# bdaiinstitute/vlfm

Hardware: NVIDIA H100
Metric: value-map steps/sec (ITM+cone-fuse) (higher is better)
Workload: dtype f16

## Files before the change

vlfm_b200/csrc/common.cuh:

```cuda
#pragma once
#include <cuda_fp16.h>
#include <cuda_runtime.h>
#include <stdint.h>
#include <stdio.h>

#include "../../include/vlfm_b200.h"

namespace vlfm {

void set_error(const char* fmt, ...);
void count_launch(unsigned n = 1);

inline int check_cuda(cudaError_t e, const char* what) {
  if (e != cudaSuccess) {
    set_error("%s: %s", what, cudaGetErrorString(e));
    return VLFM_E_CUDA;
  }
  return VLFM_OK;
}

#define VLFM_CHECK_LAUNCH(what)                                   \
  do {                                                            \
    int _rc = ::vlfm::check_cuda(cudaGetLastError(), what);       \
    if (_rc != VLFM_OK) return _rc;                               \
  } while (0)

__device__ __forceinline__ void pdl_trigger() { asm volatile("griddepcontrol.launch_dependents;" ::: "memory"); }
__device__ __forceinline__ void pdl_wait() { asm volatile("griddepcontrol.wait;" ::: "memory"); }

bool pdl_enabled();

template <typename... KArgs, typename... Args>
inline cudaError_t launch_pdl(void (*kernel)(KArgs...), dim3 grid, dim3 block, size_t smem, cudaStream_t st, Args&&... args) {
  cudaLaunchConfig_t cfg{};
  cfg.gridDim = grid; cfg.blockDim = block; cfg.dynamicSmemBytes = smem; cfg.stream = st;
  cudaLaunchAttribute attr[1];
  attr[0].id = cudaLaunchAttributeProgrammaticStreamSerialization;
  attr[0].val.programmaticStreamSerializationAllowed = 1;
  cfg.attrs = attr; cfg.numAttrs = pdl_enabled() ? 1 : 0;
  return cudaLaunchKernelEx(&cfg, kernel, static_cast<KArgs>(args)...);
}

constexpr float X2_SCALE = 2048.f;
__device__ __forceinline__ void split_x2(float y, __half& hi, __half& lo) {
  hi = __float2half_rn(y);
  lo = __float2half_rn((y - __half2float(hi)) * X2_SCALE);
}
constexpr int SK_TILE = 128;
constexpr int SK_SLAB_ROWS = SK_TILE + 2;
constexpr long long SK_SLAB = (long long)SK_SLAB_ROWS * SK_TILE;
struct SplitK {
  int splits;
  long long stride;
  int ctas, row_tiles, tiles, num_k;
  __host__ __device__ __forceinline__ int sk_begin(int c) const { return (int)((long long)c * tiles * num_k / ctas); }
  __host__ __device__ __forceinline__ int sk_owner(int it) const { return (int)(((long long)(it + 1) * ctas - 1) / ((long long)tiles * num_k)); }
};

constexpr int LN_DMAX = 1536;
int layernorm_check(const char* who, const float* d_x, const float* d_gamma, const float* d_beta, const void* d_out16, const void* d_out16_lo,
                    const float* d_out32, int D, int ldx, int ldo16, int ldo32);

__device__ __forceinline__ float ld_cg_f32(const float* p) { return __ldcg(p); }
__device__ __forceinline__ uint32_t ld_cg_u32(const uint32_t* p) { return __ldcg(p); }

}
```

vlfm_b200/csrc/gemm_wgmma.cu:

```cuda
#include <cuda.h>
#include <cuda_fp16.h>
#include <math.h>
#include <stdlib.h>

#include "common.cuh"

namespace vlfm {

constexpr int BM = 128;
constexpr int BK = 64;
constexpr int GEMM_THREADS = 384;
constexpr int GEMM_CONSUMERS = 256;

__device__ __forceinline__ uint32_t smem_u32(const void* p) { return (uint32_t)__cvta_generic_to_shared(p); }

__device__ __forceinline__ void mbar_init(uint32_t bar, uint32_t count) {
  asm volatile("mbarrier.init.shared::cta.b64 [%0], %1;" ::"r"(bar), "r"(count));
}
__device__ __forceinline__ void mbar_expect_tx(uint32_t bar, uint32_t bytes) {
  asm volatile("mbarrier.arrive.expect_tx.shared::cta.b64 _, [%0], %1;" ::"r"(bar), "r"(bytes) : "memory");
}
__device__ __forceinline__ void mbar_arrive(uint32_t bar) {
  asm volatile("mbarrier.arrive.shared::cta.b64 _, [%0];" ::"r"(bar) : "memory");
}
__device__ __forceinline__ void mbar_wait(uint32_t bar, uint32_t parity) {
  uint32_t done = 0;
  for (uint32_t spin = 0; !done; ++spin) {
    asm volatile(
        "{\n\t.reg .pred p;\n\t"
        "mbarrier.try_wait.parity.shared::cta.b64 p, [%1], %2;\n\t"
        "selp.u32 %0, 1, 0, p;\n\t}"
        : "=r"(done) : "r"(bar), "r"(parity) : "memory");
    if (spin > (1u << 26)) __trap();
  }
}
__device__ __forceinline__ void tma_load_2d(uint32_t dst, const CUtensorMap* map, int x, int y, uint32_t bar) {
  asm volatile(
      "cp.async.bulk.tensor.2d.shared::cluster.global.mbarrier::complete_tx::bytes [%0], [%1, {%3, %4}], [%2];"
      ::"r"(dst), "l"(map), "r"(bar), "r"(x), "r"(y) : "memory");
}
__device__ __forceinline__ uint64_t wgmma_desc_k128(uint32_t saddr) {
  return (uint64_t)((saddr & 0x3FFFF) >> 4) | ((uint64_t)1 << 16) | ((uint64_t)(1024 >> 4) << 32) | ((uint64_t)1 << 62);
}
__device__ __forceinline__ void wg_fence() { asm volatile("wgmma.fence.sync.aligned;" ::: "memory"); }
__device__ __forceinline__ void wg_commit() { asm volatile("wgmma.commit_group.sync.aligned;" ::: "memory"); }
template <int PENDING>
__device__ __forceinline__ void wg_wait() { asm volatile("wgmma.wait_group.sync.aligned %0;" ::"n"(PENDING) : "memory"); }

#define VLFM_D4(d, i) "+f"(d[i]), "+f"(d[i + 1]), "+f"(d[i + 2]), "+f"(d[i + 3])
#define VLFM_D16(d, i) VLFM_D4(d, i), VLFM_D4(d, i + 4), VLFM_D4(d, i + 8), VLFM_D4(d, i + 12)
template <int BN> struct Wgmma;
template <> struct Wgmma<32> {
  static __device__ __forceinline__ void mma(float (&d)[16], uint64_t a, uint64_t b, uint32_t acc) {
    asm volatile(
        "{\n\t.reg .pred p;\n\tsetp.ne.b32 p, %18, 0;\n\t"
        "wgmma.mma_async.sync.aligned.m64n32k16.f32.f16.f16 "
        "{%0,%1,%2,%3,%4,%5,%6,%7,%8,%9,%10,%11,%12,%13,%14,%15}, %16, %17, p, 1, 1, 0, 0;\n\t}"
        : VLFM_D16(d, 0) : "l"(a), "l"(b), "r"(acc));
  }
};
template <> struct Wgmma<64> {
  static __device__ __forceinline__ void mma(float (&d)[32], uint64_t a, uint64_t b, uint32_t acc) {
    asm volatile(
        "{\n\t.reg .pred p;\n\tsetp.ne.b32 p, %34, 0;\n\t"
        "wgmma.mma_async.sync.aligned.m64n64k16.f32.f16.f16 "
        "{%0,%1,%2,%3,%4,%5,%6,%7,%8,%9,%10,%11,%12,%13,%14,%15,"
        "%16,%17,%18,%19,%20,%21,%22,%23,%24,%25,%26,%27,%28,%29,%30,%31}, %32, %33, p, 1, 1, 0, 0;\n\t}"
        : VLFM_D16(d, 0), VLFM_D16(d, 16) : "l"(a), "l"(b), "r"(acc));
  }
};
template <> struct Wgmma<96> {
  static __device__ __forceinline__ void mma(float (&d)[48], uint64_t a, uint64_t b, uint32_t acc) {
    asm volatile(
        "{\n\t.reg .pred p;\n\tsetp.ne.b32 p, %50, 0;\n\t"
        "wgmma.mma_async.sync.aligned.m64n96k16.f32.f16.f16 "
        "{%0,%1,%2,%3,%4,%5,%6,%7,%8,%9,%10,%11,%12,%13,%14,%15,"
        "%16,%17,%18,%19,%20,%21,%22,%23,%24,%25,%26,%27,%28,%29,%30,%31,"
        "%32,%33,%34,%35,%36,%37,%38,%39,%40,%41,%42,%43,%44,%45,%46,%47}, %48, %49, p, 1, 1, 0, 0;\n\t}"
        : VLFM_D16(d, 0), VLFM_D16(d, 16), VLFM_D16(d, 32) : "l"(a), "l"(b), "r"(acc));
  }
};
template <> struct Wgmma<128> {
  static __device__ __forceinline__ void mma(float (&d)[64], uint64_t a, uint64_t b, uint32_t acc) {
    asm volatile(
        "{\n\t.reg .pred p;\n\tsetp.ne.b32 p, %66, 0;\n\t"
        "wgmma.mma_async.sync.aligned.m64n128k16.f32.f16.f16 "
        "{%0,%1,%2,%3,%4,%5,%6,%7,%8,%9,%10,%11,%12,%13,%14,%15,"
        "%16,%17,%18,%19,%20,%21,%22,%23,%24,%25,%26,%27,%28,%29,%30,%31,"
        "%32,%33,%34,%35,%36,%37,%38,%39,%40,%41,%42,%43,%44,%45,%46,%47,"
        "%48,%49,%50,%51,%52,%53,%54,%55,%56,%57,%58,%59,%60,%61,%62,%63}, %64, %65, p, 1, 1, 0, 0;\n\t}"
        : VLFM_D16(d, 0), VLFM_D16(d, 16), VLFM_D16(d, 32), VLFM_D16(d, 48) : "l"(a), "l"(b), "r"(acc));
  }
};
#undef VLFM_D16
#undef VLFM_D4

struct GemmArgs {
  const float* bias;
  void* out;
  int M, N, K, ldo, epi;
  int kb_per_split;
  long long split_stride;
  const __half* a_tail; int lda, tail_rows, tail_row0;
  void* out_lo;
  int a_box_rows;
  SplitK sk;
};
constexpr int GEMM_TAIL_MAX = 2;
static_assert(SK_SLAB_ROWS == BM + GEMM_TAIL_MAX && SK_TILE == BM, "stream-K slab = one 128 x 128 tile + its tail rows");
constexpr int GEMM_TAIL_KMAX = 6144;

__device__ __forceinline__ float gelu_erf(float x) { return 0.5f * x * (1.f + erff(x * 0.70710678118654752f)); }
__device__ __forceinline__ float silu(float x) { return x / (1.f + expf(-x)); }

__device__ __forceinline__ void epilogue_store2(const GemmArgs& g, int row, int n, float v0, float v1, bool pair, bool split) {
  const size_t idx = (size_t)row * g.ldo + n;
  if (g.epi == VLFM_EPI_BIAS_F16 || g.epi == VLFM_EPI_BIAS_GELU_F16 || g.epi == VLFM_EPI_BIAS_RELU_F16 || g.epi == VLFM_EPI_BIAS_GELU_F16X2) {
// ... 963 lines not shown
```

vlfm_b200/csrc/vit_ops.cu:

```cuda
#include <cuda_fp16.h>
#include <math.h>

#include "common.cuh"

namespace vlfm {

__device__ __forceinline__ uint8_t clip8(int v) {
  v >>= 22;
  return (uint8_t)(v < 0 ? 0 : (v > 255 ? 255 : v));
}

__global__ void resize_h_kernel(const uint8_t* __restrict__ in, uint8_t* __restrict__ mid, int H, int W, int OW,
                                const int* __restrict__ bounds, const int* __restrict__ kk, int ksize) {
  const int b = blockIdx.z, y = blockIdx.y;
  const int i = blockIdx.x * blockDim.x + threadIdx.x;
  if (i >= OW * 3) return;
  const int xo = i / 3, c = i - 3 * xo;
  const int x0 = bounds[2 * xo], n = bounds[2 * xo + 1];
  const uint8_t* row = in + ((size_t)b * H + y) * W * 3;
  int ss = 1 << 21;
  for (int t = 0; t < n; ++t) ss += (int)row[(x0 + t) * 3 + c] * kk[xo * ksize + t];
  mid[(((size_t)b * H + y) * OW + xo) * 3 + c] = clip8(ss);
}

__global__ void resize_v_norm_im2col_kernel(const uint8_t* __restrict__ mid, __half* __restrict__ out, int H, int OW,
                                            int OH, const int* __restrict__ bounds, const int* __restrict__ kk,
                                            int ksize, int patch, int ldk, float m0, float m1, float m2, float s0,
                                            float s1, float s2) {
  const int b = blockIdx.z, yo = blockIdx.y;
  const int i = blockIdx.x * blockDim.x + threadIdx.x;
  if (i >= OW * 3) return;
  const int xo = i / 3, c = i - 3 * xo;
  const int y0 = bounds[2 * yo], n = bounds[2 * yo + 1];
  int ss = 1 << 21;
  for (int t = 0; t < n; ++t) ss += (int)mid[(((size_t)b * H + y0 + t) * OW + xo) * 3 + c] * kk[yo * ksize + t];
  const float px = (float)clip8(ss);
  const float mean = c == 0 ? m0 : (c == 1 ? m1 : m2), sd = c == 0 ? s0 : (c == 1 ? s1 : s2);
  const float v = __fdiv_rn(__fsub_rn(__fdiv_rn(px, 255.f), mean), sd);
  const int gp = OW / patch;
  const int py = yo / patch, ky = yo - py * patch, pxi = xo / patch, kx = xo - pxi * patch;
  const size_t rowi = (size_t)b * (OH / patch) * gp + (size_t)py * gp + pxi;
  out[rowi * ldk + c * patch * patch + ky * patch + kx] = __float2half_rn(v);
}

__global__ void assemble_tokens_kernel(const float* __restrict__ patch, const float* __restrict__ cls,
                                       const float* __restrict__ pos, float* __restrict__ x, int B, int T, int D) {
  const size_t n = (size_t)B * T * D;
  for (size_t i = (size_t)blockIdx.x * blockDim.x + threadIdx.x; i < n; i += (size_t)gridDim.x * blockDim.x) {
    const int d = (int)(i % D);
    const size_t r = i / D;
    const int t = (int)(r % T), b = (int)(r / T);
    float v = t == 0 ? cls[d] : patch[((size_t)b * (T - 1) + (t - 1)) * D + d];
    x[i] = v + pos[(size_t)t * D + d];
  }
}

template <int MAXV4>
__global__ void __launch_bounds__(128)
layernorm_kernel(const float* __restrict__ x, const float* __restrict__ gamma, const float* __restrict__ beta,
                 __half* __restrict__ out16, float* __restrict__ out32, int rows, int D, int ldx, int ldo16, int ldo32,
                 float eps, __half* __restrict__ out16_lo) {
  pdl_trigger();
  const int row = blockIdx.x * 4 + (threadIdx.x >> 5), lane = threadIdx.x & 31;
  const int D4 = D >> 2;
  float4 g[MAXV4], bt[MAXV4], v[MAXV4];
#pragma unroll
  for (int i = 0; i < MAXV4; ++i) {
    const int j = lane + 32 * i;
    g[i] = j < D4 ? __ldg(reinterpret_cast<const float4*>(gamma) + j) : make_float4(0, 0, 0, 0);
    bt[i] = j < D4 ? __ldg(reinterpret_cast<const float4*>(beta) + j) : make_float4(0, 0, 0, 0);
  }
  pdl_wait();
  if (row >= rows) return;
  const float4* xr = reinterpret_cast<const float4*>(x + (size_t)row * ldx);
  float s = 0.f;
#pragma unroll
  for (int i = 0; i < MAXV4; ++i) {
    const int j = lane + 32 * i;
    v[i] = j < D4 ? xr[j] : make_float4(0, 0, 0, 0);
    s += (v[i].x + v[i].y) + (v[i].z + v[i].w);
  }
#pragma unroll
  for (int o = 16; o; o >>= 1) s += __shfl_xor_sync(0xffffffffu, s, o);
  const float mean = s / (float)D;
// ... 52 lines not shown
    s1 = sk.sk_owner((tile + 1) * sk.num_k - 1) + tile + 1;
    stride = SK_SLAB;
    off = (long long)(row - m * SK_TILE) * SK_TILE + (4 * t - nb * SK_TILE);
  }
  pdl_wait();
  float4* xr = reinterpret_cast<float4*>(x + (size_t)row * ldx);
  float4 v = on ? xr[t] : make_float4(0, 0, 0, 0);
  for (int sp0 = s0; sp0 < s1; sp0 += 4) {
    float4 pv[4];
#pragma unroll
    for (int u = 0; u < 4; ++u) {
      const float4* pr = reinterpret_cast<const float4*>(partials + (size_t)(sp0 + u) * (size_t)stride + (size_t)off);
      pv[u] = (sp0 + u < s1 && on) ? __ldcg(pr) : make_float4(0, 0, 0, 0);
    }
#pragma unroll
    for (int u = 0; u < 4; ++u)
      if (sp0 + u < s1) { v.x += pv[u].x; v.y += pv[u].y; v.z += pv[u].z; v.w += pv[u].w; }
  }
  float s = 0.f;
  if (on) { xr[t] = v; s = (v.x + v.y) + (v.z + v.w); }
#pragma unroll
  for (int o = 16; o; o >>= 1) s += __shfl_xor_sync(0xffffffffu, s, o);
  if (lane == 0) red[0][w] = s;
  __syncthreads();
  float tot = 0.f;
  for (int i = 0; i < nw; ++i) tot += red[0][i];
  const float mean = tot / (float)D;
  float q = 0.f;
  if (on) { const float a = v.x - mean, b = v.y - mean, c = v.z - mean, d = v.w - mean; q = (a * a + b * b) + (c * c + d * d); }
#pragma unroll
  for (int o = 16; o; o >>= 1) q += __shfl_xor_sync(0xffffffffu, q, o);
  if (lane == 0) red[1][w] = q;
  __syncthreads();
  float qt = 0.f;
  for (int i = 0; i < nw; ++i) qt += red[1][i];
  const float rstd = rsqrtf(qt / (float)D + eps);
  if (on) {
    float4 y;
    y.x = (v.x - mean) * rstd * g.x + bt.x;
    y.y = (v.y - mean) * rstd * g.y + bt.y;
    y.z = (v.z - mean) * rstd * g.z + bt.z;
    y.w = (v.w - mean) * rstd * g.w + bt.w;
    if (out16) {
      __half2 h0 = __floats2half2_rn(y.x, y.y), h1 = __floats2half2_rn(y.z, y.w);
      uint2 pk = make_uint2(*reinterpret_cast<uint32_t*>(&h0), *reinterpret_cast<uint32_t*>(&h1));
      *reinterpret_cast<uint2*>(out16 + (size_t)row * ldo16 + 4 * t) = pk;
      if (out16_lo) {
        const float2 f0 = __half22float2(h0), f1 = __half22float2(h1);
        __half2 l0 = __floats2half2_rn((y.x - f0.x) * X2_SCALE, (y.y - f0.y) * X2_SCALE), l1 = __floats2half2_rn((y.z - f1.x) * X2_SCALE, (y.w - f1.y) * X2_SCALE);
        uint2 pl = make_uint2(*reinterpret_cast<uint32_t*>(&l0), *reinterpret_cast<uint32_t*>(&l1));
        *reinterpret_cast<uint2*>(out16_lo + (size_t)row * ldo16 + 4 * t) = pl;
      }
    }
    if (out32) *reinterpret_cast<float4*>(out32 + (size_t)row * ldo32 + 4 * t) = y;
  }
}

__device__ __forceinline__ void mma_16816(float (&c)[4], const uint32_t (&a)[4], uint32_t b0, uint32_t b1) {
  asm volatile(
      "mma.sync.aligned.m16n8k16.row.col.f32.f16.f16.f32 {%0,%1,%2,%3}, {%4,%5,%6,%7}, {%8,%9}, {%0,%1,%2,%3};"
      : "+f"(c[0]), "+f"(c[1]), "+f"(c[2]), "+f"(c[3])
      : "r"(a[0]), "r"(a[1]), "r"(a[2]), "r"(a[3]), "r"(b0), "r"(b1));
}
__device__ __forceinline__ uint32_t pack_half2(float a, float b) {
  __half2 h = __floats2half2_rn(a, b);
  return *reinterpret_cast<uint32_t*>(&h);
}

struct AttnArgs {
  const __half* q; const __half* k; const __half* v; __half* o;
  int ldq, ldk, ldv, ldo;
  int Nq, Nk, hd, heads;
  float scale_log2;
};

constexpr int ATT_WARPS = 4;
constexpr int ATT_NKMAX = 272;

__device__ __forceinline__ void ldmatrix_x2_trans(uint32_t& r0, uint32_t& r1, const __half* p) {
  uint32_t addr = (uint32_t)__cvta_generic_to_shared(p);
  asm volatile("ldmatrix.sync.aligned.m8n8.x2.trans.shared.b16 {%0,%1}, [%2];" : "=r"(r0), "=r"(r1) : "r"(addr));
}

template <int HDP, int KH>
__global__ void __launch_bounds__(32 * (KH == 4 ? 8 : ATT_WARPS))
attention_kernel(AttnArgs a) {
  constexpr int NW = KH == 4 ? 8 : ATT_WARPS;
  constexpr int RG = NW / KH;
  constexpr int ATT_QBLK = 16 * RG;
  constexpr int KS = HDP + 8;
  extern __shared__ __align__(16) uint8_t att_smem[];
  __half* sK = reinterpret_cast<__half*>(att_smem);
  const int b = blockIdx.z, h = blockIdx.y, qb = blockIdx.x;
  const int tid = threadIdx.x, warp = tid >> 5, lane = tid & 31, g = lane >> 2, t = lane & 3;
  const int NKP = (a.Nk + 15) & ~15;
  __half* sV = sK + NKP * KS;
  pdl_trigger();
  pdl_wait();
  const __half* kbase = a.k + (size_t)b * a.Nk * a.ldk + (size_t)h * a.hd;
  const __half* vbase = a.v + (size_t)b * a.Nk * a.ldv + (size_t)h * a.hd;

  constexpr int CH = HDP / 8;
  for (int i = tid; i < NKP * CH; i += 32 * NW) {
    const int key = i / CH, c = (i - key * CH) * 8;
    const bool ok = key < a.Nk && c < a.hd;
    const __half* ksrc = ok ? kbase + (size_t)key * a.ldk + c : kbase;
    const __half* vsrc = ok ? vbase + (size_t)key * a.ldv + c : vbase;
    const uint32_t kd = (uint32_t)__cvta_generic_to_shared(sK + key * KS + c), vd = (uint32_t)__cvta_generic_to_shared(sV + key * KS + c);
    const int nbytes = ok ? 16 : 0;
    asm volatile("cp.async.cg.shared.global [%0], [%1], 16, %2;" ::"r"(kd), "l"(ksrc), "r"(nbytes) : "memory");
    asm volatile("cp.async.cg.shared.global [%0], [%1], 16, %2;" ::"r"(vd), "l"(vsrc), "r"(nbytes) : "memory");
  }
  asm volatile("cp.async.commit_group;" ::: "memory");

  const int row0 = qb * ATT_QBLK + (warp % RG) * 16;
  const int r_lo = row0 + g, r_hi = row0 + g + 8;
  const __half* qlo = a.q + ((size_t)b * a.Nq + r_lo) * a.ldq + (size_t)h * a.hd;
  const __half* qhi = a.q + ((size_t)b * a.Nq + r_hi) * a.ldq + (size_t)h * a.hd;
  uint32_t qf[HDP / 16][4];
#pragma unroll
  for (int kk = 0; kk < HDP / 16; ++kk) {
    const int c0 = kk * 16 + 2 * t, c1 = c0 + 8;
    qf[kk][0] = (r_lo < a.Nq && c0 < a.hd) ? *reinterpret_cast<const uint32_t*>(qlo + c0) : 0u;
    qf[kk][1] = (r_hi < a.Nq && c0 < a.hd) ? *reinterpret_cast<const uint32_t*>(qhi + c0) : 0u;
    qf[kk][2] = (r_lo < a.Nq && c1 < a.hd) ? *reinterpret_cast<const uint32_t*>(qlo + c1) : 0u;
    qf[kk][3] = (r_hi < a.Nq && c1 < a.hd) ? *reinterpret_cast<const uint32_t*>(qhi + c1) : 0u;
  }
  asm volatile("cp.async.wait_group 0;" ::: "memory");
  __syncthreads();

  float o[HDP / 8][4];
#pragma unroll
  for (int i = 0; i < HDP / 8; ++i) { o[i][0] = o[i][1] = o[i][2] = o[i][3] = 0.f; }
  float m_lo = -INFINITY, m_hi = -INFINITY, l_lo = 0.f, l_hi = 0.f;

  const int part = warp / RG, tiles = NKP >> 4, tbase = tiles / KH, trem = tiles % KH;
  const int k_begin = 16 * (part * tbase + min(part, trem)), k_end = k_begin + 16 * (tbase + (part < trem ? 1 : 0));
  for (int kb = k_begin; kb < k_end; kb += 64) {
    const int ntiles = min(8, (k_end - kb) >> 3);
    float s[8][4];
#pragma unroll
    for (int j = 0; j < 8; ++j) {
      s[j][0] = s[j][1] = s[j][2] = s[j][3] = 0.f;
      if (j < ntiles) {
        const __half* kr = sK + (kb + j * 8 + g) * KS + 2 * t;
#pragma unroll
        for (int kk = 0; kk < HDP / 16; ++kk) {
          uint32_t b0 = *reinterpret_cast<const uint32_t*>(kr + kk * 16);
          uint32_t b1 = *reinterpret_cast<const uint32_t*>(kr + kk * 16 + 8);
          mma_16816(s[j], qf[kk], b0, b1);
        }
      }
    }
    float bm_lo = -INFINITY, bm_hi = -INFINITY;
#pragma unroll
    for (int j = 0; j < 8; ++j) {
      const int key = kb + j * 8 + 2 * t;
#pragma unroll
      for (int e = 0; e < 4; ++e) {
        const bool ok = (j < ntiles) && (key + (e & 1) < a.Nk);
        s[j][e] = ok ? s[j][e] * a.scale_log2 : -INFINITY;
      }
      bm_lo = fmaxf(bm_lo, fmaxf(s[j][0], s[j][1]));
      bm_hi = fmaxf(bm_hi, fmaxf(s[j][2], s[j][3]));
    }
    bm_lo = fmaxf(bm_lo, __shfl_xor_sync(0xffffffffu, bm_lo, 1));
    bm_lo = fmaxf(bm_lo, __shfl_xor_sync(0xffffffffu, bm_lo, 2));
    bm_hi = fmaxf(bm_hi, __shfl_xor_sync(0xffffffffu, bm_hi, 1));
    bm_hi = fmaxf(bm_hi, __shfl_xor_sync(0xffffffffu, bm_hi, 2));
    const float mn_lo = fmaxf(m_lo, bm_lo), mn_hi = fmaxf(m_hi, bm_hi);
    const float ref_lo = mn_lo == -INFINITY ? 0.f : mn_lo, ref_hi = mn_hi == -INFINITY ? 0.f : mn_hi;
    const float al_lo = exp2f(m_lo - ref_lo), al_hi = exp2f(m_hi - ref_hi);
    m_lo = mn_lo; m_hi = mn_hi;
    float sum_lo = 0.f, sum_hi = 0.f;
#pragma unroll
    for (int j = 0; j < 8; ++j) {
      s[j][0] = exp2f(s[j][0] - ref_lo); s[j][1] = exp2f(s[j][1] - ref_lo);
      s[j][2] = exp2f(s[j][2] - ref_hi); s[j][3] = exp2f(s[j][3] - ref_hi);
      sum_lo += s[j][0] + s[j][1]; sum_hi += s[j][2] + s[j][3];
    }
    l_lo = l_lo * al_lo + sum_lo; l_hi = l_hi * al_hi + sum_hi;
#pragma unroll
    for (int i = 0; i < HDP / 8; ++i) { o[i][0] *= al_lo; o[i][1] *= al_lo; o[i][2] *= al_hi; o[i][3] *= al_hi; }
#pragma unroll
    for (int p = 0; p < 4; ++p) {
      if (2 * p < ntiles) {
        uint32_t pa[4];
        pa[0] = pack_half2(s[2 * p][0], s[2 * p][1]);
        pa[1] = pack_half2(s[2 * p][2], s[2 * p][3]);
        pa[2] = pack_half2(s[2 * p + 1][0], s[2 * p + 1][1]);
        pa[3] = pack_half2(s[2 * p + 1][2], s[2 * p + 1][3]);
        const __half* vr = sV + (kb + p * 16 + (lane & 15)) * KS;
#pragma unroll
        for (int i = 0; i < HDP / 8; ++i) {
          uint32_t b0, b1;
          ldmatrix_x2_trans(b0, b1, vr + i * 8);
          mma_16816(o[i], pa, b0, b1);
        }
      }
    }
  }
  l_lo += __shfl_xor_sync(0xffffffffu, l_lo, 1); l_lo += __shfl_xor_sync(0xffffffffu, l_lo, 2);
  l_hi += __shfl_xor_sync(0xffffffffu, l_hi, 1); l_hi += __shfl_xor_sync(0xffffffffu, l_hi, 2);

  if (KH == 1) {
    const float inv_lo = 1.f / l_lo, inv_hi = 1.f / l_hi;
    __half* olo = a.o + ((size_t)b * a.Nq + r_lo) * a.ldo + (size_t)h * a.hd;
    __half* ohi = a.o + ((size_t)b * a.Nq + r_hi) * a.ldo + (size_t)h * a.hd;
#pragma unroll
    for (int i = 0; i < HDP / 8; ++i) {
      const int c = i * 8 + 2 * t;
      if (c < a.hd) {
        if (r_lo < a.Nq) *reinterpret_cast<uint32_t*>(olo + c) = pack_half2(o[i][0] * inv_lo, o[i][1] * inv_lo);
        if (r_hi < a.Nq) *reinterpret_cast<uint32_t*>(ohi + c) = pack_half2(o[i][2] * inv_hi, o[i][3] * inv_hi);
      }
    }
    return;
  }
  __syncthreads();
  float* mrg = reinterpret_cast<float*>(att_smem);
  constexpr int MW = HDP / 8 * 4 + 4;
  if (warp >= RG) {
// ... 236 lines not shown

namespace vlfm {
int layernorm_check(const char* who, const float* d_x, const float* d_gamma, const float* d_beta, const void* d_out16, const void* d_out16_lo,
                    const float* d_out32, int D, int ldx, int ldo16, int ldo32) {
  if (D > LN_DMAX) { set_error("%s: D=%d too large (max %d)", who, D, LN_DMAX); return VLFM_E_UNSUPPORTED; }
  if ((D & 3) || (ldx & 3) || (ldo16 & 3) || (ldo32 & 3)) { set_error("%s: D and strides must be multiples of 4", who); return VLFM_E_UNSUPPORTED; }
  if (((uintptr_t)d_x & 15) || ((uintptr_t)d_gamma & 15) || ((uintptr_t)d_beta & 15) || ((uintptr_t)d_out32 & 15) ||
      ((uintptr_t)d_out16 & 7) || ((uintptr_t)d_out16_lo & 7)) {
    set_error("%s: x, gamma, beta, out32 must be 16-byte aligned, the fp16 outputs 8-byte aligned", who); return VLFM_E_INVALID; }
  return VLFM_OK;
}
}

static int layernorm_impl(const float* d_x, const float* d_gamma, const float* d_beta, void* d_out16, void* d_out16_lo, float* d_out32,
                          int rows, int D, int ldx, int ldo16, int ldo32, float eps, void* stream) {
  __half* lo16 = (__half*)d_out16_lo;
  if (!d_x || !d_gamma || !d_beta || (!d_out16 && !d_out32) || rows < 1 || D < 1) { set_error("vlfm_layernorm: bad argument"); return VLFM_E_INVALID; }
  if (int rc = layernorm_check("vlfm_layernorm", d_x, d_gamma, d_beta, d_out16, d_out16_lo, d_out32, D, ldx, ldo16, ldo32)) return rc;
  cudaStream_t st = (cudaStream_t)stream;
  const dim3 grid((rows + 3) / 4);
  cudaError_t e;
  __half* o16 = (__half*)d_out16;
  if (D <= 128 * 2) e = launch_pdl(layernorm_kernel<2>, grid, dim3(128), 0, st, d_x, d_gamma, d_beta, o16, d_out32, rows, D, ldx, ldo16, ldo32, eps, lo16);
  else if (D <= 128 * 6) e = launch_pdl(layernorm_kernel<6>, grid, dim3(128), 0, st, d_x, d_gamma, d_beta, o16, d_out32, rows, D, ldx, ldo16, ldo32, eps, lo16);
  else e = launch_pdl(layernorm_kernel<12>, grid, dim3(128), 0, st, d_x, d_gamma, d_beta, o16, d_out32, rows, D, ldx, ldo16, ldo32, eps, lo16);
  { int rc = check_cuda(e, "layernorm_kernel"); if (rc) return rc; }
  count_launch();
  return VLFM_OK;
}
extern "C" int vlfm_layernorm(const float* d_x, const float* d_gamma, const float* d_beta, void* d_out16, float* d_out32,
                              int rows, int D, int ldx, int ldo16, int ldo32, float eps, void* stream) {
  return layernorm_impl(d_x, d_gamma, d_beta, d_out16, nullptr, d_out32, rows, D, ldx, ldo16, ldo32, eps, stream);
}
extern "C" int vlfm_layernorm_x2(const float* d_x, const float* d_gamma, const float* d_beta, void* d_out_hi, void* d_out_lo, float* d_out32,
                                 int rows, int D, int ldx, int ldo16, int ldo32, float eps, void* stream) {
  if (!d_out_hi || !d_out_lo) { set_error("vlfm_layernorm_x2: null output"); return VLFM_E_INVALID; }
  return layernorm_impl(d_x, d_gamma, d_beta, d_out_hi, d_out_lo, d_out32, rows, D, ldx, ldo16, ldo32, eps, stream);
}

namespace vlfm {
int layernorm_reduce_impl(float* d_x, const float* d_partials, const SplitK& sk, const float* d_gamma,
                          const float* d_beta, void* d_out16, void* d_out16_lo, float* d_out32, int rows, int D, int ldx, int ldo16, int ldo32,
                          float eps, void* stream) {
  __half* lo16 = (__half*)d_out16_lo;
  if (!d_x || !d_partials || !d_gamma || !d_beta || (!d_out16 && !d_out32) || rows < 1 || D < 1 || sk.splits < 0 || sk.splits > 16 ||
      (sk.splits == 0 && (sk.ctas < 1 || sk.row_tiles < 1 || sk.tiles != sk.row_tiles * ((D + SK_TILE - 1) / SK_TILE) || sk.num_k < 1))) {
    set_error("vlfm_layernorm_reduce: bad argument"); return VLFM_E_INVALID; }
  if (int rc = layernorm_check("vlfm_layernorm_reduce", d_x, d_gamma, d_beta, d_out16, d_out16_lo, d_out32, D, ldx, ldo16, ldo32)) return rc;
  if (sk.stride & 3) { set_error("vlfm_layernorm_reduce: D and strides must be multiples of 4"); return VLFM_E_UNSUPPORTED; }
  if ((uintptr_t)d_partials & 15) { set_error("vlfm_layernorm_reduce: partials must be 16-byte aligned"); return VLFM_E_INVALID; }
  cudaStream_t st = (cudaStream_t)stream;
  const dim3 grid(rows);
  __half* o16 = (__half*)d_out16;
  cudaError_t e;
  const int threads = (((D >> 2) + 31) / 32) * 32;
  e = launch_pdl(layernorm_reduce_kernel, grid, dim3(threads), 0, st, d_x, d_partials, sk, d_gamma, d_beta, o16, d_out32, rows, D, ldx, ldo16, ldo32, eps, lo16);
  { int rc = check_cuda(e, "layernorm_reduce_kernel"); if (rc) return rc; }
  count_launch();
  return VLFM_OK;
}
}
extern "C" int vlfm_layernorm_reduce(float* d_x, const float* d_partials, int splits, long long split_stride, const float* d_gamma,
                                     const float* d_beta, void* d_out16, float* d_out32, int rows, int D, int ldx, int ldo16, int ldo32,
                                     float eps, void* stream) {
  if (splits < 1) { set_error("vlfm_layernorm_reduce: bad argument"); return VLFM_E_INVALID; }
  return layernorm_reduce_impl(d_x, d_partials, SplitK{splits, split_stride}, d_gamma, d_beta, d_out16, nullptr, d_out32, rows, D, ldx, ldo16, ldo32, eps, stream);
}
extern "C" int vlfm_layernorm_reduce_x2(float* d_x, const float* d_partials, int splits, long long split_stride, const float* d_gamma,
                                        const float* d_beta, void* d_out_hi, void* d_out_lo, float* d_out32, int rows, int D, int ldx, int ldo16,
                                        int ldo32, float eps, void* stream) {
  if (!d_out_hi || !d_out_lo) { set_error("vlfm_layernorm_reduce_x2: null output"); return VLFM_E_INVALID; }
  if (splits < 1) { set_error("vlfm_layernorm_reduce_x2: bad argument"); return VLFM_E_INVALID; }
  return layernorm_reduce_impl(d_x, d_partials, SplitK{splits, split_stride}, d_gamma, d_beta, d_out_hi, d_out_lo, d_out32, rows, D, ldx, ldo16, ldo32, eps, stream);
}

extern "C" int vlfm_attention_f16(const void* d_q, const void* d_k, const void* d_v, void* d_o, int B, int heads, int Nq,
                                  int Nk, int hd, int ldq, int ldk, int ldv, int ldo, float scale, void* stream) {
  if (!d_q || !d_k || !d_v || !d_o || B < 1 || heads < 1 || Nq < 1 || Nk < 1) { set_error("vlfm_attention_f16: bad argument"); return VLFM_E_INVALID; }
  if (Nk > ATT_NKMAX || hd > 96 || (hd & 7) || (ldq & 7) || (ldk & 7) || (ldv & 7) || (ldo & 1) || B > 65535) {
    set_error("vlfm_attention_f16: unsupported shape (Nk<=%d, hd<=96 and %%8==0, strides %%8==0)", ATT_NKMAX); return VLFM_E_UNSUPPORTED; }
  AttnArgs a{(const __half*)d_q, (const __half*)d_k, (const __half*)d_v, (__half*)d_o, ldq, ldk, ldv, ldo, Nq, Nk, hd, heads,
             scale * 1.4426950408889634f};
  cudaStream_t st = (cudaStream_t)stream;
  const long items = (long)B * heads * ((Nq + 31) / 32);
  const bool big = items > 2 * 264;
  static int kh4 = -1;
  if (kh4 < 0) { const char* e = getenv("VLFM_ATT_KH4"); kh4 = e ? atoi(e) : 1; }
  const bool quad = !big && kh4 && items <= 264 && Nk >= 64;
  const int qblk = big ? 64 : 32;
  dim3 grid((Nq + qblk - 1) / qblk, heads, B);
  const size_t nkp = ((size_t)Nk + 15) & ~(size_t)15;
  static bool cfg = false;
  if (!cfg) {
    int rc = check_cuda(cudaFuncSetAttribute(attention_kernel<64, 1>, cudaFuncAttributeMaxDynamicSharedMemorySize, 2 * ATT_NKMAX * (64 + 8) * 2), "attr(attention)");
    if (!rc) rc = check_cuda(cudaFuncSetAttribute(attention_kernel<64, 2>, cudaFuncAttributeMaxDynamicSharedMemorySize, 2 * ATT_NKMAX * (64 + 8) * 2), "attr(attention)");
    if (!rc) rc = check_cuda(cudaFuncSetAttribute(attention_kernel<96, 1>, cudaFuncAttributeMaxDynamicSharedMemorySize, 2 * ATT_NKMAX * (96 + 8) * 2), "attr(attention)");
    if (!rc) rc = check_cuda(cudaFuncSetAttribute(attention_kernel<96, 2>, cudaFuncAttributeMaxDynamicSharedMemorySize, 2 * ATT_NKMAX * (96 + 8) * 2), "attr(attention)");
    if (!rc) rc = check_cuda(cudaFuncSetAttribute(attention_kernel<64, 4>, cudaFuncAttributeMaxDynamicSharedMemorySize, 2 * ATT_NKMAX * (64 + 8) * 2), "attr(attention)");
    if (!rc) rc = check_cuda(cudaFuncSetAttribute(attention_kernel<96, 4>, cudaFuncAttributeMaxDynamicSharedMemorySize, 2 * ATT_NKMAX * (96 + 8) * 2), "attr(attention)");
    if (rc) return rc;
    cfg = true;
  }
  const int hdp = hd <= 64 ? 64 : 96;
  size_t sm = 2 * nkp * (hdp + 8) * 2;
  if (sm < 6 * 52 * 32 * 4) sm = 6 * 52 * 32 * 4;
  cudaError_t e;
  if (quad) e = hdp == 64 ? launch_pdl(attention_kernel<64, 4>, grid, dim3(256), sm, st, a) : launch_pdl(attention_kernel<96, 4>, grid, dim3(256), sm, st, a);
  else if (hdp == 64) e = big ? launch_pdl(attention_kernel<64, 1>, grid, dim3(32 * ATT_WARPS), sm, st, a) : launch_pdl(attention_kernel<64, 2>, grid, dim3(32 * ATT_WARPS), sm, st, a);
  else e = big ? launch_pdl(attention_kernel<96, 1>, grid, dim3(32 * ATT_WARPS), sm, st, a) : launch_pdl(attention_kernel<96, 2>, grid, dim3(32 * ATT_WARPS), sm, st, a);
  { int rc = check_cuda(e, "attention_kernel"); if (rc) return rc; }
  count_launch();
  return VLFM_OK;
}

extern "C" int vlfm_attention_f32(const float* d_q, const float* d_k, const float* d_v, void* d_o_hi, void* d_o_lo, int B, int heads, int Nq,
                                  int Nk, int hd, int ldq, int ldk, int ldv, int ldo, float scale, void* stream) {
  if (!d_q || !d_k || !d_v || !d_o_hi || !d_o_lo || B < 1 || heads < 1 || Nq < 1 || Nk < 1) { set_error("vlfm_attention_f32: bad argument"); return VLFM_E_INVALID; }
  if (Nk > ATT32_NKMAX || (hd != 32 && hd != 64) || (ldk & 3) || (ldv & 3) || B > 65535) {
    set_error("vlfm_attention_f32: unsupported shape (Nk<=%d, hd in {32,64}, strides %%4==0)", ATT32_NKMAX); return VLFM_E_UNSUPPORTED; }
  const size_t smem = ((((size_t)Nk * (hd + 1) + 3) & ~(size_t)3) + (size_t)Nk * hd + 8 * hd + 8 * (size_t)Nk) * 4;
  static size_t cfg32 = 0, cfg64 = 0;
  size_t& cfg = hd == 32 ? cfg32 : cfg64;
  if (smem > 48 * 1024 && smem > cfg) {
    int rc = hd == 32 ? check_cuda(cudaFuncSetAttribute(attention_f32_kernel<32>, cudaFuncAttributeMaxDynamicSharedMemorySize, (int)smem), "attr(attention_f32)")
                      : check_cuda(cudaFuncSetAttribute(attention_f32_kernel<64>, cudaFuncAttributeMaxDynamicSharedMemorySize, (int)smem), "attr(attention_f32)");
    if (rc) return rc; cfg = smem;
  }
  int z = (Nq + 7) / 8;
  while (z > 1 && (long)heads * B * z > 2 * 132) --z;
  const dim3 grid(heads, B, z);
  cudaError_t e = hd == 32 ? launch_pdl(attention_f32_kernel<32>, grid, dim3(256), smem, (cudaStream_t)stream, d_q, d_k, d_v, (__half*)d_o_hi, (__half*)d_o_lo,
                                        ldq, ldk, ldv, ldo, Nq, Nk, scale)
                           : launch_pdl(attention_f32_kernel<64>, grid, dim3(256), smem, (cudaStream_t)stream, d_q, d_k, d_v, (__half*)d_o_hi, (__half*)d_o_lo,
                                        ldq, ldk, ldv, ldo, Nq, Nk, scale);
  { int rc = check_cuda(e, "attention_f32_kernel"); if (rc) return rc; }
  count_launch();
  return VLFM_OK;
}

extern "C" int vlfm_split_x2(const float* d_src, void* d_hi, void* d_lo, long long n, void* stream) {
  if (!d_src || !d_lo || n < 4 || (n & 3) || ((uintptr_t)d_src & 15) || ((uintptr_t)d_lo & 7) || ((uintptr_t)d_hi & 7)) {
    set_error("vlfm_split_x2: bad argument (n %% 4 == 0, aligned pointers)"); return VLFM_E_INVALID; }
  long blocks = (n / 4 + 255) / 256; if (blocks > 132 * 8) blocks = 132 * 8;
  cudaError_t e = launch_pdl(split_x2_kernel, dim3((unsigned)blocks), dim3(256), 0, (cudaStream_t)stream, d_src, (__half*)d_hi, (__half*)d_lo, (long)(n / 4));
  { int rc = check_cuda(e, "split_x2_kernel"); if (rc) return rc; }
  count_launch();
  return VLFM_OK;
}

extern "C" int vlfm_itc_head_multi(const float* d_proj, const float* d_text, float* d_out, int B, int P, int Q, int D, int ldo,
                                   void* stream) {
  if (!d_proj || !d_text || !d_out || B < 1 || P < 1 || Q < 1 || D < 1 || ldo < P || (size_t)Q * sizeof(float) > 48 * 1024) {
    set_error("vlfm_itc_head_multi: bad argument (B, P, Q, D >= 1, ldo >= P, Q <= 12288)"); return VLFM_E_INVALID; }
  itc_head_kernel<<<B, 256, Q * sizeof(float), (cudaStream_t)stream>>>(d_proj, d_text, d_out, P, Q, D, ldo);
  VLFM_CHECK_LAUNCH("itc_head_kernel");
  count_launch();
  return VLFM_OK;
}

extern "C" int vlfm_itc_head(const float* d_proj, const float* d_text, float* d_out, int B, int Q, int D, void* stream) {
  if (!d_proj || !d_text || !d_out || B < 1) { set_error("vlfm_itc_head: bad argument"); return VLFM_E_INVALID; }
  return vlfm_itc_head_multi(d_proj, d_text, d_out, B, 1, Q, D, 1, stream);
}
```

Measured before the change: 227.3.

## Add batch-1 attention variant with 16 warps and mbarrier-staged K/V chunks

Adds a small-batch attention kernel variant that uses 512 threads covering 64 query rows and splits the keys into four parts. Q is staged into shared memory and read back with ldmatrix. K/V are loaded in four cp.async chunks, each signalling its own mbarrier, so each key-split warp group can start as soon as its chunk lands instead of waiting for the whole K/V load. The point is more parallelism and load/compute overlap when there are few (batch, head, query-block) items. It adds extra shared memory for Q and barriers, reloads Q fragments inside the loop, and adds a getenv call on every invocation.

```diff
diff --git a/vlfm_b200/csrc/common.cuh b/vlfm_b200/csrc/common.cuh
--- a/vlfm_b200/csrc/common.cuh
+++ b/vlfm_b200/csrc/common.cuh
@@ -29,6 +29,23 @@
 __device__ __forceinline__ void pdl_wait() { asm volatile("griddepcontrol.wait;" ::: "memory"); }
 
 bool pdl_enabled();
+
+__device__ __forceinline__ uint32_t smem_u32(const void* p) { return (uint32_t)__cvta_generic_to_shared(p); }
+
+__device__ __forceinline__ void mbar_init(uint32_t bar, uint32_t count) {
+  asm volatile("mbarrier.init.shared::cta.b64 [%0], %1;" ::"r"(bar), "r"(count));
+}
+__device__ __forceinline__ void mbar_wait(uint32_t bar, uint32_t parity) {
+  uint32_t done = 0;
+  for (uint32_t spin = 0; !done; ++spin) {
+    asm volatile(
+        "{\n\t.reg .pred p;\n\t"
+        "mbarrier.try_wait.parity.shared::cta.b64 p, [%1], %2;\n\t"
+        "selp.u32 %0, 1, 0, p;\n\t}"
+        : "=r"(done) : "r"(bar), "r"(parity) : "memory");
+    if (spin > (1u << 26)) __trap();
+  }
+}
 
 template <typename... KArgs, typename... Args>
 inline cudaError_t launch_pdl(void (*kernel)(KArgs...), dim3 grid, dim3 block, size_t smem, cudaStream_t st, Args&&... args) {
diff --git a/vlfm_b200/csrc/gemm_wgmma.cu b/vlfm_b200/csrc/gemm_wgmma.cu
--- a/vlfm_b200/csrc/gemm_wgmma.cu
+++ b/vlfm_b200/csrc/gemm_wgmma.cu
@@ -12,27 +12,11 @@
 constexpr int GEMM_THREADS = 384;
 constexpr int GEMM_CONSUMERS = 256;
 
-__device__ __forceinline__ uint32_t smem_u32(const void* p) { return (uint32_t)__cvta_generic_to_shared(p); }
-
-__device__ __forceinline__ void mbar_init(uint32_t bar, uint32_t count) {
-  asm volatile("mbarrier.init.shared::cta.b64 [%0], %1;" ::"r"(bar), "r"(count));
-}
 __device__ __forceinline__ void mbar_expect_tx(uint32_t bar, uint32_t bytes) {
   asm volatile("mbarrier.arrive.expect_tx.shared::cta.b64 _, [%0], %1;" ::"r"(bar), "r"(bytes) : "memory");
 }
 __device__ __forceinline__ void mbar_arrive(uint32_t bar) {
   asm volatile("mbarrier.arrive.shared::cta.b64 _, [%0];" ::"r"(bar) : "memory");
-}
-__device__ __forceinline__ void mbar_wait(uint32_t bar, uint32_t parity) {
-  uint32_t done = 0;
-  for (uint32_t spin = 0; !done; ++spin) {
-    asm volatile(
-        "{\n\t.reg .pred p;\n\t"
-        "mbarrier.try_wait.parity.shared::cta.b64 p, [%1], %2;\n\t"
-        "selp.u32 %0, 1, 0, p;\n\t}"
-        : "=r"(done) : "r"(bar), "r"(parity) : "memory");
-    if (spin > (1u << 26)) __trap();
-  }
 }
 __device__ __forceinline__ void tma_load_2d(uint32_t dst, const CUtensorMap* map, int x, int y, uint32_t bar) {
   asm volatile(
diff --git a/vlfm_b200/csrc/vit_ops.cu b/vlfm_b200/csrc/vit_ops.cu
--- a/vlfm_b200/csrc/vit_ops.cu
+++ b/vlfm_b200/csrc/vit_ops.cu
@@ -1,5 +1,7 @@
 #include <cuda_fp16.h>
 #include <math.h>
+#include <stdlib.h>
+#include <string.h>
 
 #include "common.cuh"
 
@@ -218,10 +220,55 @@
   asm volatile("ldmatrix.sync.aligned.m8n8.x2.trans.shared.b16 {%0,%1}, [%2];" : "=r"(r0), "=r"(r1) : "r"(addr));
 }
 
-template <int HDP, int KH>
-__global__ void __launch_bounds__(32 * (KH == 4 ? 8 : ATT_WARPS))
+constexpr int ATT_B1_ROWS = 64;
+constexpr int ATT_B1_THREADS = 512;
+constexpr int ATT_B1_BARS = 5;
+
+__host__ __device__ constexpr int attn_b1_bar_offset(int nkp, int hdp) {
+  return (2 * nkp + ATT_B1_ROWS) * (hdp + 8) * 2 > 12 * (hdp / 2 + 4) * 32 * 4 ? (2 * nkp + ATT_B1_ROWS) * (hdp + 8) * 2
+                                                                              : 12 * (hdp / 2 + 4) * 32 * 4;
+}
+
+__device__ __forceinline__ void ldmatrix_x4(uint32_t (&r)[4], const __half* p) {
+  asm volatile("ldmatrix.sync.aligned.m8n8.x4.shared.b16 {%0,%1,%2,%3}, [%4];"
+               : "=r"(r[0]), "=r"(r[1]), "=r"(r[2]), "=r"(r[3]) : "r"(smem_u32(p)));
+}
+
+template <int HDP>
+__device__ __forceinline__ void attn_b1_stage(const AttnArgs& a, uint8_t* smem, __half* sK, __half* sV, const __half* kbase,
+                                              const __half* vbase, int NKP, int qb, int tid) {
+  constexpr int KS = HDP + 8, CH = HDP / 8;
+  const uint32_t bars = smem_u32(smem + attn_b1_bar_offset(NKP, HDP));
+  if (tid == 0) {
+    for (int i = 0; i < ATT_B1_BARS; ++i) mbar_init(bars + 8 * i, ATT_B1_THREADS);
+    asm volatile("fence.mbarrier_init.release.cluster;" ::: "memory");
+  }
+  __syncthreads();
+  auto copy_rows = [&](__half* dst, const __half* src, int ld, int r0, int r1, int rlim) {
+    for (int i = r0 * CH + tid; i < r1 * CH; i += ATT_B1_THREADS) {
+      const int r = i / CH, c = (i - r * CH) * 8;
+      const bool ok = r < rlim && c < a.hd;
+      const __half* p = ok ? src + (size_t)r * ld + c : src;
+      asm volatile("cp.async.cg.shared.global [%0], [%1], 16, %2;" ::"r"(smem_u32(dst + r * KS + c)), "l"(p), "r"(ok ? 16 : 0) : "memory");
+    }
+  };
+  const __half* qbase = a.q + ((size_t)blockIdx.z * a.Nq + (size_t)qb * ATT_B1_ROWS) * a.ldq + (size_t)blockIdx.y * a.hd;
+  copy_rows(sV + NKP * KS, qbase, a.ldq, 0, ATT_B1_ROWS, min(ATT_B1_ROWS, a.Nq - qb * ATT_B1_ROWS));
+  asm volatile("cp.async.mbarrier.arrive.noinc.shared::cta.b64 [%0];" ::"r"(bars) : "memory");
+  const int tiles = NKP >> 4, tbase = tiles / 4, trem = tiles % 4;
+  for (int p = 0; p < 4; ++p) {
+    const int k0 = 16 * (p * tbase + min(p, trem)), k1 = k0 + 16 * (tbase + (p < trem ? 1 : 0));
+    copy_rows(sK, kbase, a.ldk, k0, k1, a.Nk);
+    copy_rows(sV, vbase, a.ldv, k0, k1, a.Nk);
+    asm volatile("cp.async.mbarrier.arrive.noinc.shared::cta.b64 [%0];" ::"r"(bars + 8 * (1 + p)) : "memory");
+  }
+}
+
+template <int HDP, int KH, bool B1 = false>
+__global__ void __launch_bounds__(32 * (B1 ? 16 : (KH == 4 ? 8 : ATT_WARPS)))
 attention_kernel(AttnArgs a) {
-  constexpr int NW = KH == 4 ? 8 : ATT_WARPS;
+  static_assert(!B1 || KH == 4, "the batch-1 variant splits the keys in four");
+  constexpr int NW = B1 ? 16 : (KH == 4 ? 8 : ATT_WARPS);
   constexpr int RG = NW / KH;
   constexpr int ATT_QBLK = 16 * RG;
   constexpr int KS = HDP + 8;
@@ -237,6 +284,9 @@
   const __half* vbase = a.v + (size_t)b * a.Nk * a.ldv + (size_t)h * a.hd;
 
   constexpr int CH = HDP / 8;
+  if constexpr (B1) {
+    attn_b1_stage<HDP>(a, att_smem, sK, sV, kbase, vbase, NKP, qb, tid);
+  } else {
   for (int i = tid; i < NKP * CH; i += 32 * NW) {
     const int key = i / CH, c = (i - key * CH) * 8;
     const bool ok = key < a.Nk && c < a.hd;
@@ -248,12 +298,16 @@
     asm volatile("cp.async.cg.shared.global [%0], [%1], 16, %2;" ::"r"(vd), "l"(vsrc), "r"(nbytes) : "memory");
   }
   asm volatile("cp.async.commit_group;" ::: "memory");
+  }
 
   const int row0 = qb * ATT_QBLK + (warp % RG) * 16;
   const int r_lo = row0 + g, r_hi = row0 + g + 8;
+  uint32_t qf[HDP / 16][4];
+  if constexpr (B1) {
+    mbar_wait(smem_u32(att_smem + attn_b1_bar_offset(NKP, HDP)), 0);
+  } else {
   const __half* qlo = a.q + ((size_t)b * a.Nq + r_lo) * a.ldq + (size_t)h * a.hd;
   const __half* qhi = a.q + ((size_t)b * a.Nq + r_hi) * a.ldq + (size_t)h * a.hd;
-  uint32_t qf[HDP / 16][4];
 #pragma unroll
   for (int kk = 0; kk < HDP / 16; ++kk) {
     const int c0 = kk * 16 + 2 * t, c1 = c0 + 8;
@@ -264,6 +318,7 @@
   }
   asm volatile("cp.async.wait_group 0;" ::: "memory");
   __syncthreads();
+  }
 
   float o[HDP / 8][4];
 #pragma unroll
@@ -272,8 +327,14 @@
 
   const int part = warp / RG, tiles = NKP >> 4, tbase = tiles / KH, trem = tiles % KH;
   const int k_begin = 16 * (part * tbase + min(part, trem)), k_end = k_begin + 16 * (tbase + (part < trem ? 1 : 0));
+  if constexpr (B1) mbar_wait(smem_u32(att_smem + attn_b1_bar_offset(NKP, HDP)) + 8 * (1 + part), 0);
   for (int kb = k_begin; kb < k_end; kb += 64) {
     const int ntiles = min(8, (k_end - kb) >> 3);
+    if constexpr (B1) {
+      const __half* qr = sV + NKP * KS + ((warp % RG) * 16 + (lane & 15)) * KS + (lane >> 4) * 8;
+#pragma unroll
+      for (int kk = 0; kk < HDP / 16; ++kk) ldmatrix_x4(qf[kk], qr + kk * 16);
+    }
     float s[8][4];
 #pragma unroll
     for (int j = 0; j < 8; ++j) {
@@ -676,6 +737,29 @@
   AttnArgs a{(const __half*)d_q, (const __half*)d_k, (const __half*)d_v, (__half*)d_o, ldq, ldk, ldv, ldo, Nq, Nk, hd, heads,
              scale * 1.4426950408889634f};
   cudaStream_t st = (cudaStream_t)stream;
+  const char* impl = getenv("VLFM_ATT_IMPL");
+  const bool force_legacy = impl && !strcmp(impl, "legacy"), force_b1 = impl && !strcmp(impl, "b1");
+  if (impl && impl[0] && !force_legacy && !force_b1) { set_error("vlfm_attention_f16: VLFM_ATT_IMPL=%s (legacy or b1)", impl); return VLFM_E_INVALID; }
+  const size_t nkp = ((size_t)Nk + 15) & ~(size_t)15;
+  const int hdp = hd <= 64 ? 64 : 96;
+  const long items64 = (long)B * heads * ((Nq + ATT_B1_ROWS - 1) / ATT_B1_ROWS);
+  if (force_b1 || (!force_legacy && items64 <= 132 && Nk >= 64)) {
+    static bool cfg_b1 = false;
+    if (!cfg_b1) {
+      const int mx = attn_b1_bar_offset(ATT_NKMAX, 96) + 8 * ATT_B1_BARS;
+      int rc = check_cuda(cudaFuncSetAttribute(attention_kernel<64, 4, true>, cudaFuncAttributeMaxDynamicSharedMemorySize, mx), "attr(attention b1)");
+      if (!rc) rc = check_cuda(cudaFuncSetAttribute(attention_kernel<96, 4, true>, cudaFuncAttributeMaxDynamicSharedMemorySize, mx), "attr(attention b1)");
+      if (rc) return rc;
+      cfg_b1 = true;
+    }
+    const size_t sm = attn_b1_bar_offset((int)nkp, hdp) + 8 * ATT_B1_BARS;
+    const dim3 grid((Nq + ATT_B1_ROWS - 1) / ATT_B1_ROWS, heads, B);
+    cudaError_t e = hdp == 64 ? launch_pdl(attention_kernel<64, 4, true>, grid, dim3(ATT_B1_THREADS), sm, st, a)
+                              : launch_pdl(attention_kernel<96, 4, true>, grid, dim3(ATT_B1_THREADS), sm, st, a);
+    { int rc = check_cuda(e, "attention_kernel (batch 1)"); if (rc) return rc; }
+    count_launch();
+    return VLFM_OK;
+  }
   const long items = (long)B * heads * ((Nq + 31) / 32);
   const bool big = items > 2 * 264;
   static int kh4 = -1;
@@ -683,7 +767,6 @@
   const bool quad = !big && kh4 && items <= 264 && Nk >= 64;
   const int qblk = big ? 64 : 32;
   dim3 grid((Nq + qblk - 1) / qblk, heads, B);
-  const size_t nkp = ((size_t)Nk + 15) & ~(size_t)15;
   static bool cfg = false;
   if (!cfg) {
     int rc = check_cuda(cudaFuncSetAttribute(attention_kernel<64, 1>, cudaFuncAttributeMaxDynamicSharedMemorySize, 2 * ATT_NKMAX * (64 + 8) * 2), "attr(attention)");
@@ -695,7 +778,6 @@
     if (rc) return rc;
     cfg = true;
   }
-  const int hdp = hd <= 64 ? 64 : 96;
   size_t sm = 2 * nkp * (hdp + 8) * 2;
   if (sm < 6 * 52 * 32 * 4) sm = 6 * 52 * 32 * 4;
   cudaError_t e;
```

Result: faster. 234.7, median of 6 (+3.3%).
